# PRBonn/lidar_transfer

Measured on AMD Instinct MI355X. Metric: Mrays/sec, one new ~1M-triangle mesh per scan -> 64x2048 range/label image, higher is better.
Workload: dtype f32; 1 GPU; C2: 64x2048 rays vs 999788-triangle synthetic scene (fov 3.0/-25.0); 1 step = 64 scans, each a new mesh; 48 scenes cycled; parallelism=scan-parallel x1, scans_in_flight=24, scans_per_call=8

## Files before the change

### lidar_transfer_amd/csrc/lt_scatter.hip

```cpp
#include "lt_internal.h"
#include <math.h>
#include <stdlib.h>
#include <string.h>
#include "lt_normalize.h"

#define LT_PI_F 3.14159265358979f
#define LT_BIN_SLACK 4e-3f
#define LT_EMPTY_KEY 0xFFFFFFFFFFFFFFFFull

struct rs_params {
  int nb_az, nb_el;
  float az_scale;
  float az_off;
  float el_lo, el_scale;
  float dev_az, dev_el;
  float dev_fit[2];
  float el_c0, el_c1, az_c0, az_c1;
};

__device__ __forceinline__ float rs_az_off(float phi0, float az_scale) {
  if (!(phi0 == phi0)) return 0.f;
  const float x0 = (phi0 + LT_PI_F) * az_scale;
  return x0 - floorf(x0 + 0.5f);
}

__global__ __launch_bounds__(256) void k_rs_dirs(const float* __restrict__ rays, int n, unsigned flags,
                                                 float4* __restrict__ dirs, float2* __restrict__ ang,
                                                 float* __restrict__ partial) {
  __shared__ float red[4][2];
  float lo = INFINITY, hi = -INFINITY;
  for (int i = blockIdx.x * 256 + threadIdx.x; i < n; i += gridDim.x * 256) {
    const float rx = rays[3 * (size_t)i], ry = rays[3 * (size_t)i + 1], rz = rays[3 * (size_t)i + 2];
    const float D = (rx * rx + ry * ry) + rz * rz;
    const float r0 = lt_rsqrt_seed(D, flags);
    const float r = (1.5f * r0) + (((D * -0.5f) * r0) * (r0 * r0));
    const float dx = rx * r, dy = ry * r, dz = rz * r;
    dirs[i] = make_float4(dx, dy, dz, 0.f);
    const float phi = atan2f(dy, dx), th = atan2f(dz, sqrtf(dx * dx + dy * dy));
    ang[i] = make_float2(phi, th);
    if (th == th) { lo = fminf(lo, th); hi = fmaxf(hi, th); }
  }
#pragma unroll
  for (int o = 32; o > 0; o >>= 1) {
    lo = fminf(lo, __shfl_xor(lo, o, 64));
    hi = fmaxf(hi, __shfl_xor(hi, o, 64));
  }
  if ((threadIdx.x & 63) == 0) { red[threadIdx.x >> 6][0] = lo; red[threadIdx.x >> 6][1] = hi; }
  __syncthreads();
  if (threadIdx.x == 0) {
    partial[2 * blockIdx.x] = fminf(fminf(red[0][0], red[1][0]), fminf(red[2][0], red[3][0]));
    partial[2 * blockIdx.x + 1] = fmaxf(fmaxf(red[0][1], red[1][1]), fmaxf(red[2][1], red[3][1]));
  }
}

__global__ __launch_bounds__(256) void k_rs_fit(const float2* __restrict__ ang, int n, int nb_az0,
                                                rs_params* __restrict__ prm) {
  const float phi0 = n > 0 ? ang[0].x : 0.f;
  float dev[2] = {0.f, 0.f};
  for (int k = 0; k < 2; ++k) {
    const int K = nb_az0 - k;
    if (K < 1) continue;
    const float sc = (float)K / (2.0f * LT_PI_F), off = rs_az_off(phi0, sc);
    for (int i = blockIdx.x * 256 + threadIdx.x; i < n; i += gridDim.x * 256) {
      const float phi = ang[i].x;
      if (phi == phi) {
        const float x = (phi + LT_PI_F) * sc - off;
        dev[k] = fmaxf(dev[k], fabsf(x - floorf(x + 0.5f)));
      }
    }
  }
#pragma unroll
  for (int o = 32; o > 0; o >>= 1) {
    dev[0] = fmaxf(dev[0], __shfl_xor(dev[0], o, 64));
    dev[1] = fmaxf(dev[1], __shfl_xor(dev[1], o, 64));
  }
  if ((threadIdx.x & 63) == 0) {
    atomicMax((int*)&prm->dev_fit[0], __float_as_int(dev[0]));
    atomicMax((int*)&prm->dev_fit[1], __float_as_int(dev[1]));
  }
}

__global__ __launch_bounds__(256) void k_rs_keys(const float2* __restrict__ ang, int n, int nb_az, int nb_el, int refit,
                                                 const float* __restrict__ partial, rs_params* __restrict__ prm,
                                                 uint32_t* __restrict__ keys, uint32_t* __restrict__ vals) {
  __shared__ float red[4][2];
  float lo = partial[2 * threadIdx.x], hi = partial[2 * threadIdx.x + 1];
#pragma unroll
  for (int o = 32; o > 0; o >>= 1) {
    lo = fminf(lo, __shfl_xor(lo, o, 64));
    hi = fmaxf(hi, __shfl_xor(hi, o, 64));
  }
  if ((threadIdx.x & 63) == 0) { red[threadIdx.x >> 6][0] = lo; red[threadIdx.x >> 6][1] = hi; }
  __syncthreads();
  lo = fminf(fminf(red[0][0], red[1][0]), fminf(red[2][0], red[3][0]));
  hi = fmaxf(fmaxf(red[0][1], red[1][1]), fmaxf(red[2][1], red[3][1]));
  if (!(lo <= hi)) { lo = 0.f; hi = 0.f; }
  const int nb_max = nb_az;
  if (refit && nb_az >= 5 && prm->dev_fit[1] + 0.01f < prm->dev_fit[0]) nb_az -= 1;
  rs_params p;
  p.nb_az = nb_az; p.nb_el = nb_el;
  p.az_scale = (float)nb_az / (2.0f * LT_PI_F);
  p.az_off = rs_az_off(n > 0 ? ang[0].x : 0.f, p.az_scale);
  p.el_lo = lo;
  p.el_scale = (nb_el > 1 && hi > lo) ? (float)(nb_el - 1) / (hi - lo) : 0.f;
  if (blockIdx.x == 0 && threadIdx.x == 0) {
    prm->nb_az = p.nb_az; prm->nb_el = p.nb_el;
    prm->az_scale = p.az_scale; prm->az_off = p.az_off; prm->el_lo = p.el_lo; prm->el_scale = p.el_scale;
  }
  const int i = blockIdx.x * 256 + threadIdx.x;
  float dev_a = 0.f, dev_e = 0.f;
  if (i < n) {
    const float2 a = ang[i];
    uint32_t key = (uint32_t)nb_max * (uint32_t)nb_el;
    if (a.x == a.x && a.y == a.y) {
      const float x = (a.x + LT_PI_F) * p.az_scale - p.az_off, y = (a.y - p.el_lo) * p.el_scale;
      const float cx = floorf(x + 0.5f);
      const float cy = fminf(fmaxf(floorf(y + 0.5f), 0.f), (float)(nb_el - 1));
      dev_a = fabsf(x - cx);
      dev_e = fabsf(y - cy);
      int ia = (int)cx;
      if (ia < 0) ia += nb_az;
      else if (ia >= nb_az) ia -= nb_az;
      ia = min(max(ia, 0), nb_az - 1);
      key = (uint32_t)cy * (uint32_t)nb_az + (uint32_t)ia;
    }
    keys[i] = key;
    vals[i] = (uint32_t)i;
  }
#pragma unroll
  for (int o = 32; o > 0; o >>= 1) {
    dev_a = fmaxf(dev_a, __shfl_xor(dev_a, o, 64));
    dev_e = fmaxf(dev_e, __shfl_xor(dev_e, o, 64));
  }
  if ((threadIdx.x & 63) == 0) {
    atomicMax((int*)&prm->dev_az, __float_as_int(dev_a));
    atomicMax((int*)&prm->dev_el, __float_as_int(dev_e));
  }
}

__global__ __launch_bounds__(256) void k_rs_starts(const uint32_t* __restrict__ keys, int n, int nbins,
                                                   int* __restrict__ bin_start) {
  const int p = blockIdx.x * 256 + threadIdx.x;
  if (p > n) return;
  const int lo = p == 0 ? 0 : (int)min(keys[p - 1], (uint32_t)nbins) + 1;
  const int hi = p == n ? nbins : (int)min(keys[p], (uint32_t)nbins);
  for (int b = lo; b <= hi; ++b) bin_start[b] = p;
}

struct tri_rec {
  float v0x, v0y, v0z, e1x, e1y, e1z, e2x, e2y, e2z;
};

__device__ __forceinline__ float sc_mt(const tri_rec& T, float ox, float oy, float oz, float dx, float dy, float dz) {
  const float eps = 0.000001f;
  const float hx = dy * T.e2z - dz * T.e2y, hy = dz * T.e2x - dx * T.e2z, hz = dx * T.e2y - dy * T.e2x;
  const float a = (T.e1x * hx + T.e1y * hy) + T.e1z * hz;
  if (a < eps && a > -eps) return NAN;
  const float inv_a = lt_rcp_ieee(a);
  const float sx = ox - T.v0x, sy = oy - T.v0y, sz = oz - T.v0z;
  const float u = ((sx * hx + sy * hy) + sz * hz) * inv_a;
  if (u < 0 || u > 1) return NAN;
  const float qx = sy * T.e1z - sz * T.e1y, qy = sz * T.e1x - sx * T.e1z, qz = sx * T.e1y - sy * T.e1x;
  const float v = ((dx * qx + dy * qy) + dz * qz) * inv_a;
  if (v < 0 || u + v > 1) return NAN;
  const float t = ((T.e2x * qx + T.e2y * qy) + T.e2z * qz) * inv_a;
  if (t < eps) return NAN;
  return t;
}

__device__ __forceinline__ float f_rcp(float x) { return __builtin_amdgcn_rcpf(x); }
__device__ __forceinline__ float f_sqrt(float x) { return __builtin_amdgcn_sqrtf(x); }
__device__ __forceinline__ float f_atan2(float y, float x) {
#pragma clang fp contract(fast)
  const float ax = fabsf(x), ay = fabsf(y);
  const float mx = fmaxf(ax, ay), mn = fminf(ax, ay);
  const float a = mx > 0.f ? mn * f_rcp(mx) : 0.f;
  const float q = a * a;
  float r = a * (0.99997726f + q * (-0.33262347f + q * (0.19354346f + q * (-0.11643287f + q * (0.05265332f + q * -0.01172120f)))));
  r = ay > ax ? 1.57079632679f - r : r;
  r = x < 0.f ? 3.14159265359f - r : r;
  return y < 0.f ? -r : r;
}

__device__ __forceinline__ void f_atan_pair(float za, float ra, float zb, float rb, float& tha, float& thb) {
#pragma clang fp contract(fast)
  const float ta = za * f_rcp(ra), tb = zb * f_rcp(rb);
  const bool easy = fabsf(ta) <= 1.0f && fabsf(tb) <= 1.0f;
  if (__ballot(!easy) == 0ull) {
    const float qa = ta * ta, qb = tb * tb;
    tha = ta * (0.99997726f + qa * (-0.33262347f + qa * (0.19354346f + qa * (-0.11643287f + qa * (0.05265332f + qa * -0.01172120f)))));
    thb = tb * (0.99997726f + qb * (-0.33262347f + qb * (0.19354346f + qb * (-0.11643287f + qb * (0.05265332f + qb * -0.01172120f)))));
  } else {
    tha = f_atan2(za, ra);
    thb = f_atan2(zb, rb);
  }
}

__device__ __forceinline__ float seg_dist2d_sq(float ax, float ay, float bx, float by) {
#pragma clang fp contract(fast)
  const float ex = bx - ax, ey = by - ay;
  const float l2 = ex * ex + ey * ey;
  float t = l2 > 0.f ? -(ax * ex + ay * ey) * f_rcp(l2) : 0.f;
  t = fminf(fmaxf(t, 0.f), 1.f);
  const float cx = ax + t * ex, cy = ay + t * ey;
  return cx * cx + cy * cy;
}

template <class T>
__device__ __forceinline__ unsigned byte_off(unsigned elem) {
  if (sizeof(T) == 12) {
    unsigned r;
    asm("v_lshl_add_u32 %0, %1, 3, %2" : "=v"(r) : "v"(elem), "v"(elem << 2));
    return r;
  }
  return elem * (unsigned)sizeof(T);
}
template <bool WIDE, class T>
__device__ __forceinline__ const T* at(const T* base, unsigned elem) {
  return WIDE ? base + (size_t)elem : (const T*)((const char*)base + byte_off<T>(elem));
}
template <bool WIDE, class T>
__device__ __forceinline__ T* at(T* base, unsigned elem) {
  return WIDE ? base + (size_t)elem : (T*)((char*)base + byte_off<T>(elem));
}
struct f3 { float x, y, z; };
struct i3 { int x, y, z; };

struct bin_rect { int a0, na, e0, e1; };

__device__ __forceinline__ bin_rect tri_bins(const rs_params& P, float x0, float y0, float z0, float x1, float y1,
                                             float z1, float x2, float y2, float z2, float e1x, float e1y, float e2x,
                                             float e2y) {
#pragma clang fp contract(fast)
  bin_rect R;
  R.na = 0;
  const float q0 = x0 * x0 + y0 * y0, q1 = x1 * x1 + y1 * y1, q2 = x2 * x2 + y2 * y2;
  if (!(q0 + q1 + q2 < 1e36f && fabsf(z0) + fabsf(z1) + fabsf(z2) < 1e18f)) {
    const float sum = ((x0 + y0) + (z0 + x1)) + ((y1 + z1) + (x2 + y2)) + z2;
    const float asum = ((fabsf(x0) + fabsf(y0)) + (fabsf(z0) + fabsf(x1))) + ((fabsf(y1) + fabsf(z1)) + (fabsf(x2) + fabsf(y2))) + fabsf(z2);
    if (sum != sum || asum == INFINITY) return R;
    R.e0 = 0; R.e1 = P.nb_el - 1; R.a0 = 0; R.na = P.nb_az;
    return R;
  }
  const float rho_max2 = fmaxf(q0, fmaxf(q1, q2));
  const float rho_max = f_sqrt(rho_max2);
  const float zmin = fminf(z0, fminf(z1, z2)), zmax = fmaxf(z0, fmaxf(z1, z2));
  const float c0 = x0 * y1 - x1 * y0, c1 = x1 * y2 - x2 * y1, c2 = x2 * y0 - x0 * y2;
  const float tol = 1e-6f * rho_max2 + 1e-12f;
  const float cmin = fminf(c0, fminf(c1, c2)), cmax = fmaxf(c0, fmaxf(c1, c2));
  const bool outside = cmin < -tol && cmax > tol;
  bool edge_on = cmin >= -tol && cmax <= tol;
  const float e12x = e2x - e1x, e12y = e2y - e1y;
  const float lmax2 = fmaxf(e1x * e1x + e1y * e1y, fmaxf(e12x * e12x + e12y * e12y, e2x * e2x + e2y * e2y));
  const float qmin = fminf(q0, fminf(q1, q2));
  float rho_edges2;
  if (__ballot(!(lmax2 <= 0.01f * qmin)) == 0ull) {
    rho_edges2 = qmin - 0.25f * lmax2;
  } else {
    rho_edges2 =
        fminf(seg_dist2d_sq(x0, y0, x1, y1), fminf(seg_dist2d_sq(x1, y1, x2, y2), seg_dist2d_sq(x2, y2, x0, y0)));
  }
  const float rho_edges = f_sqrt(rho_edges2);
  const float rho_tiny = 1e-4f * rho_max + 1e-6f;
  if (!outside && rho_edges2 > 4.0f * lmax2) edge_on = true;
  const bool pierced = !(outside || (edge_on && rho_edges > rho_tiny));
  const float rho_min = pierced ? 0.f : rho_edges;
  const float z_near = __builtin_amdgcn_fmed3f(zmin, 0.f, zmax);
  const float dlo2 = fmaxf((pierced ? 0.f : rho_edges2) + z_near * z_near, 0.0025f);
  const float pad = 3e-4f + 2e-4f * __builtin_amdgcn_rsqf(dlo2);
  const float pad_az = 3e-4f + 2e-4f * __builtin_amdgcn_rsqf(fmaxf(rho_edges2, 0.0025f));
  float th_hi, th_lo;
  f_atan_pair(zmax, zmax > 0.f ? rho_min : rho_max, zmin, zmin < 0.f ? rho_min : rho_max, th_hi, th_lo);
  th_hi += pad;
  th_lo -= pad;
  const float fe0 = ceilf(th_lo * P.el_scale + P.el_c0), fe1 = floorf(th_hi * P.el_scale + P.el_c1);
  if (!(fe1 >= 0.f) || !(fe0 <= (float)(P.nb_el - 1)) || !(fe0 <= fe1)) return R;
  R.e0 = (int)fmaxf(fe0, 0.f);
  R.e1 = (int)fminf(fe1, (float)(P.nb_el - 1));
  if (pierced || rho_min <= rho_tiny || P.nb_az < 4) {
    R.a0 = 0;
    R.na = P.nb_az;
    return R;
  }
  float a_lo, a_hi;
  if (!edge_on) {
    const bool l0 = c0 >= 0.f && c2 <= 0.f, l1 = c1 >= 0.f && c0 <= 0.f;
    const bool h0 = c0 <= 0.f && c2 >= 0.f, h1 = c1 <= 0.f && c0 >= 0.f;
    a_lo = f_atan2(l0 ? y0 : (l1 ? y1 : y2), l0 ? x0 : (l1 ? x1 : x2));
    a_hi = f_atan2(h0 ? y0 : (h1 ? y1 : y2), h0 ? x0 : (h1 ? x1 : x2));
    if (a_hi < a_lo) a_hi += 2.0f * LT_PI_F;
  } else {
    const float p0 = f_atan2(y0, x0), p1 = f_atan2(y1, x1), p2 = f_atan2(y2, x2);
    const float lo = fminf(p0, fminf(p1, p2)), hi = fmaxf(p0, fmaxf(p1, p2));
    const float mid = (p0 + p1 + p2) - lo - hi;
    const float g0 = mid - lo, g1 = hi - mid, g2 = 2.0f * LT_PI_F - (hi - lo);
    if (g2 >= g0 && g2 >= g1) { a_lo = lo; a_hi = hi; }
    else if (g0 >= g1) { a_lo = mid; a_hi = lo + 2.0f * LT_PI_F; }
    else { a_lo = hi; a_hi = mid + 2.0f * LT_PI_F; }
  }
  a_lo -= pad_az;
  a_hi += pad_az;
  const float fa0 = ceilf(a_lo * P.az_scale + P.az_c0);
  const float fa1 = floorf(a_hi * P.az_scale + P.az_c1);
  const int na = (int)(fa1 - fa0) + 1;
  if (!(na >= 1)) return R;
  if (na >= P.nb_az) { R.a0 = 0; R.na = P.nb_az; return R; }
  int a0 = (int)fa0;
  if (a0 < 0) a0 += P.nb_az;
  else if (a0 >= P.nb_az) a0 -= P.nb_az;
  R.a0 = a0;
  R.na = na;
  return R;
}

#define LT_GRID_EMPTY (-1)
#define LT_GRID_MULTI (-2)
template <bool WIDE>
__device__ __forceinline__ void sc_hit(float t, int ray, int face, unsigned long long* __restrict__ cell) {
  if (t < 999999999.f) atomicMin(at<WIDE>(cell, (unsigned)ray), ((unsigned long long)__float_as_uint(t) << 32) | (unsigned)face);
}
template <bool WIDE>
__device__ __forceinline__ void sc_test_cell(const tri_rec& T, int face, const float4 g,
                                             const float4* __restrict__ sdirs, float ox, float oy, float oz,
                                             unsigned long long* __restrict__ cell, unsigned& n_tests) {
  const int w = __float_as_int(g.w);
  if (w != LT_GRID_MULTI) {
    n_tests += w >= 0 ? 1u : 0u;
    sc_hit<WIDE>(sc_mt(T, ox, oy, oz, g.x, g.y, g.z), w, face, cell);
  } else {
    for (int k = __float_as_int(g.x), e = __float_as_int(g.y); k < e; ++k) {
      const float4 d = *at<WIDE>(sdirs, (unsigned)k);
      ++n_tests;
      sc_hit<WIDE>(sc_mt(T, ox, oy, oz, d.x, d.y, d.z), __float_as_int(d.w), face, cell);
    }
  }
}

__global__ __launch_bounds__(256) void k_rs_sortdirs(const float4* __restrict__ dirs,
                                                     const uint32_t* __restrict__ bin_rays, int n,
                                                     float4* __restrict__ sdirs) {
  const int k = blockIdx.x * 256 + threadIdx.x;
  if (k >= n) return;
  const int ray = (int)bin_rays[k];
  float4 d = dirs[ray];
  d.w = __int_as_float(ray);
  sdirs[k] = d;
}

__global__ __launch_bounds__(256) void k_rs_grid(const int* __restrict__ bin_start,
                                                 const float4* __restrict__ sdirs, int nbins,
                                                 float4* __restrict__ grid) {
  const int b = blockIdx.x * 256 + threadIdx.x;
  if (b >= nbins) return;
  const int s = bin_start[b], e = bin_start[b + 1];
  float4 g = make_float4(0.f, 0.f, 0.f, __int_as_float(LT_GRID_EMPTY));
  if (e - s == 1) g = sdirs[s];
  else if (e - s > 1) g = make_float4(__int_as_float(s), __int_as_float(e), 0.f, __int_as_float(LT_GRID_MULTI));
  grid[b] = g;
}

#define LT_SC_BIG 512
#define LT_SC_CAP_SINGLE 1536
#define LT_SC_CAP_BATCH 8192
#ifndef LT_SC_SLICE
#define LT_SC_SLICE 512
#endif

#ifndef LT_SC_T
#define LT_SC_T 448
#endif
#define LT_SC_T2 (LT_SC_T - 256)
static_assert(LT_SC_T >= 256 && LT_SC_T <= 512 && LT_SC_T2 % 64 == 0, "LT_SC_T: 256, 320, 384, 448 or 512");

struct sc_shared {
  float4 q0[LT_SC_T], q1[LT_SC_T];
  float2 q2[LT_SC_T];
  unsigned pre[513];
  unsigned wsum[4];
  int kept;
};

struct sc_one { int cnt; unsigned a0; };

template <bool PUSH>
__device__ __forceinline__ sc_one sc_record_into(float4* s_q0, float4* s_q1, float2* s_q2, int slot, int f, const f3 A,
                                                 const f3 Bv, const f3 C, float ox, float oy, float oz, const rs_params& P,
                                                 int* __restrict__ large, int* __restrict__ large_count) {
  sc_one r;
  r.cnt = 0; r.a0 = 0;
  const float v0x = A.x, v0y = A.y, v0z = A.z, v1x = Bv.x, v1y = Bv.y, v1z = Bv.z;
  const float v2x = C.x, v2y = C.y, v2z = C.z;
  const float e1x = v1x - v0x, e1y = v1y - v0y, e2x = v2x - v0x, e2y = v2y - v0y;
  const bin_rect R = tri_bins(P, v0x - ox, v0y - oy, v0z - oz, v1x - ox, v1y - oy, v1z - oz, v2x - ox, v2y - oy,
                              v2z - oz, e1x, e1y, e2x, e2y);
  if (R.na > 0) {
    const int c32 = R.na * (R.e1 - R.e0 + 1);
    if (c32 > LT_SC_BIG) {
      if (PUSH) large[atomicAdd(large_count, 1)] = f;
    } else {
      r.cnt = c32;
      r.a0 = (unsigned)R.a0;
      s_q0[slot] = make_float4(v0x, v0y, v0z, e1x);
      s_q1[slot] = make_float4(e1y, v1z - v0z, e2x, e2y);
      s_q2[slot] = make_float2(v2z - v0z, __int_as_float((R.na - 1) | (R.e0 << 9)));
    }
  }
  return r;
}
template <bool PUSH>
__device__ __forceinline__ sc_one sc_record(sc_shared& S, int slot, int f, const f3 A, const f3 Bv, const f3 C, float ox,
                                            float oy, float oz, const rs_params& P, int* __restrict__ large,
                                            int* __restrict__ large_count) {
  return sc_record_into<PUSH>(S.q0, S.q1, S.q2, slot, f, A, Bv, C, ox, oy, oz, P, large, large_count);
}

template <bool PUSH, bool WIDE>
__device__ __forceinline__ void sc_setup(sc_shared& S, const float* __restrict__ verts, const int* __restrict__ faces,
                                         int n_verts, int n_faces, int first, float ox, float oy, float oz,
                                         const rs_params& P, int* __restrict__ large, int* __restrict__ large_count,
                                         unsigned* __restrict__ flags, sc_one& rA, sc_one& rB) {
  const int tid = threadIdx.x;
  rA.cnt = 0; rA.a0 = 0; rB.cnt = 0; rB.a0 = 0;
  const int fA = first + tid, fB = first + 256 + tid;
  const bool hasA = fA < n_faces, hasB = LT_SC_T2 > 0 && tid < LT_SC_T2 && fB < n_faces;
  if (n_verts <= 0) {
    if (PUSH && (hasA || hasB)) atomicOr(flags, LT_FLAG_BAD_INDEX);
    return;
  }
  const i3 iA = *at<WIDE>((const i3*)faces, (unsigned)(hasA ? fA : 0));
  i3 iB = iA;
  if (LT_SC_T2 > 0) iB = *at<WIDE>((const i3*)faces, (unsigned)(hasB ? fB : 0));
  const unsigned nv = (unsigned)n_verts;
  const bool okA = hasA && (unsigned)iA.x < nv && (unsigned)iA.y < nv && (unsigned)iA.z < nv;
  const bool okB = hasB && (unsigned)iB.x < nv && (unsigned)iB.y < nv && (unsigned)iB.z < nv;
  const f3 A0 = *at<WIDE>((const f3*)verts, okA ? (unsigned)iA.x : 0u);
  const f3 A1 = *at<WIDE>((const f3*)verts, okA ? (unsigned)iA.y : 0u);
  const f3 A2 = *at<WIDE>((const f3*)verts, okA ? (unsigned)iA.z : 0u);
  f3 B0 = A0, B1 = A1, B2 = A2;
  if (LT_SC_T2 > 0) {
    B0 = *at<WIDE>((const f3*)verts, okB ? (unsigned)iB.x : 0u);
    B1 = *at<WIDE>((const f3*)verts, okB ? (unsigned)iB.y : 0u);
    B2 = *at<WIDE>((const f3*)verts, okB ? (unsigned)iB.z : 0u);
  }
  if (PUSH && ((hasA && !okA) || (hasB && !okB))) atomicOr(flags, LT_FLAG_BAD_INDEX);
  if (okA) rA = sc_record<PUSH>(S, tid, fA, A0, A1, A2, ox, oy, oz, P, large, large_count);
  if (LT_SC_T2 > 0 && okB) rB = sc_record<PUSH>(S, 256 + tid, fB, B0, B1, B2, ox, oy, oz, P, large, large_count);
}

__device__ __forceinline__ void sc_prefix(sc_shared& S, const sc_one rA, const sc_one rB, int& preA, int& preB, int& total) {
  const int tid = threadIdx.x, lane = tid & 63, wave = tid >> 6;
  unsigned inc = (unsigned)rA.cnt | ((unsigned)rB.cnt << 16);
  asm volatile(
      "s_nop 1\n\tv_add_u32_dpp %0, %0, %0 row_shr:1 row_mask:0xf bank_mask:0xf bound_ctrl:0\n\t"
      "s_nop 1\n\tv_add_u32_dpp %0, %0, %0 row_shr:2 row_mask:0xf bank_mask:0xf bound_ctrl:0\n\t"
      "s_nop 1\n\tv_add_u32_dpp %0, %0, %0 row_shr:4 row_mask:0xf bank_mask:0xf bound_ctrl:0\n\t"
      "s_nop 1\n\tv_add_u32_dpp %0, %0, %0 row_shr:8 row_mask:0xf bank_mask:0xf bound_ctrl:0\n\t"
      "s_nop 1\n\tv_add_u32_dpp %0, %0, %0 row_bcast:15 row_mask:0xa bank_mask:0xf\n\t"
      "s_nop 1\n\tv_add_u32_dpp %0, %0, %0 row_bcast:31 row_mask:0xc bank_mask:0xf\n\t"
      "s_nop 1"
      : "+v"(inc));
  if (lane == 63) S.wsum[wave] = inc;
  __syncthreads();
  int woffA = 0, woffB = 0, totA = 0, totB = 0;
#pragma unroll
  for (int w = 0; w < 4; ++w) {
    const unsigned ws = S.wsum[w];
    const int a = (int)(ws & 0xFFFFu), b = (int)(ws >> 16);
    if (w < wave) { woffA += a; woffB += b; }
    totA += a; totB += b;
  }
  total = totA + totB;
  preA = woffA + (int)(inc & 0xFFFFu) - rA.cnt;
  preB = totA + woffB + (int)(inc >> 16) - rB.cnt;
  S.pre[tid] = ((unsigned)preA << 13) | rA.a0;
  if (LT_SC_T2 > 0 && tid < LT_SC_T2) S.pre[256 + tid] = ((unsigned)preB << 13) | rB.a0;
  else S.pre[256 + tid] = (256 + tid == LT_SC_T) ? ((unsigned)total << 13) : 0xFFFFFFFFu;
  if (tid == 255) S.pre[512] = LT_SC_T == 512 ? ((unsigned)total << 13) : 0xFFFFFFFFu;
}

template <bool COUNT, bool WIDE, int NT, int NE>
__device__ __forceinline__ void sc_round_robin(const unsigned* s_pre, const float4* s_q0, const float4* s_q1,
                                               const float2* s_q2, const rs_params& P, const float4* __restrict__ grid,
                                               const float4* __restrict__ sdirs, unsigned long long* __restrict__ cell,
                                               int first_face, int c_begin, int c_end, int tix, float ox, float oy, float oz,
                                               unsigned& n_tests, unsigned& n_cand) {
  auto ldu = [](const unsigned* arr, unsigned j4) { return *(const unsigned*)((const char*)arr + j4); };
  auto ldq = [](const float4* arr, unsigned j4) { return *(const float4*)((const char*)arr + 4u * j4); };
  auto ld2 = [](const float2* arr, unsigned j4) { return *(const float2*)((const char*)arr + 2u * j4); };
  const unsigned pre0 = s_pre[0];
  auto locate = [&](int c, unsigned& j4, float2& q2) -> int {
    const unsigned ck = ((unsigned)c << 13) | 0x1FFFu;
    j4 = 0;
    unsigned base = pre0;
#pragma unroll
    for (unsigned step4 = 2u * NE; step4 >= 4; step4 >>= 1) {
      const unsigned v = ldu(s_pre, j4 + step4);
      const bool take = v <= ck;
      j4 = take ? j4 + step4 : j4;
      base = take ? v : base;
    }
    const int local = c - (int)(base >> 13);
    q2 = ld2(s_q2, j4);
    const int pk = __float_as_int(q2.y);
    const int na = (pk & 511) + 1;
    const int row = (int)(((float)local + 0.5f) * f_rcp((float)na));
    int az = (int)(base & 0x1FFFu) + (local - __mul24(row, na));
    if (az >= P.nb_az) az -= P.nb_az;
    return __mul24((pk >> 9) + row, P.nb_az) + az;
  };
  int c = c_begin + tix;
  if (c < c_end) {
    unsigned j4;
    float2 q2;
    float4 g = *at<false>(grid, (unsigned)locate(c, j4, q2));
    for (;;) {
      const int cn = c + NT;
      unsigned jn4 = 0;
      float2 q2n = make_float2(0.f, 0.f);
      float4 gn = make_float4(0.f, 0.f, 0.f, 0.f);
      if (__ballot(cn < c_end) != 0ull) gn = *at<false>(grid, (unsigned)locate(min(cn, c_end - 1), jn4, q2n));
      const float4 q0 = ldq(s_q0, j4), q1 = ldq(s_q1, j4);
      tri_rec T;
      T.v0x = q0.x; T.v0y = q0.y; T.v0z = q0.z;
      T.e1x = q0.w; T.e1y = q1.x; T.e1z = q1.y;
      T.e2x = q1.z; T.e2y = q1.w; T.e2z = q2.x;
      if (COUNT) ++n_cand;
      sc_test_cell<WIDE>(T, first_face + (int)(j4 >> 2), g, sdirs, ox, oy, oz, cell, n_tests);
      if (cn >= c_end) break;
      c = cn; j4 = jn4; g = gn; q2 = q2n;
    }
  }
}

template <bool COUNT>
__device__ __forceinline__ void sc_count(unsigned n_tests, unsigned n_cand, unsigned long long* __restrict__ counters) {
  if (COUNT) {
    unsigned long long vt = n_tests, vc = n_cand;
#pragma unroll
    for (int o = 32; o > 0; o >>= 1) { vt += __shfl_xor(vt, o, 64); vc += __shfl_xor(vc, o, 64); }
    if ((threadIdx.x & 63) == 0) { atomicAdd(&counters[1], vt); atomicAdd(&counters[0], vc); }
  }
}

#ifndef LT_SC_MAX_BATCH
#define LT_SC_MAX_BATCH 8
#endif
struct sc_job {
  const float* verts; const int* faces; const int* colors; const float* rem;
  rs_params P; const float4* grid; const float4* sdirs; const float4* dirs;
  unsigned long long* cell; int* large; int* large_count; int2* slices;
  unsigned* flags; unsigned long long* counters;
  float* endpoints; int* endcolors; float* range; float* endrem; int* tri;
  float ox, oy, oz;
  int n_verts, n_faces, n_rays, cap_slices;
  unsigned out_flags;
};
struct sc_batch {
  int n;
  int tris_blocks, resolve_blocks;
  int cap;
  int rest_blocks;
  int tris_block0[LT_SC_MAX_BATCH];
  int resolve_block0[LT_SC_MAX_BATCH];
  sc_job job[LT_SC_MAX_BATCH];
};
__device__ __forceinline__ int sc_find_job(const int (&block0)[LT_SC_MAX_BATCH], int block) {
  int j = 0;
#pragma unroll
  for (int k = 1; k < LT_SC_MAX_BATCH; ++k) j += block >= block0[k] ? 1 : 0;
  return j;
}


template <bool COUNT, bool WIDE>
__global__ __launch_bounds__(256) void k_sc_tris(const sc_batch B) {
  __shared__ sc_shared S;
  const int j = sc_find_job(B.tris_block0, (int)blockIdx.x);
  const sc_job& J = B.job[j];
  const int lb = (int)blockIdx.x - B.tris_block0[j];
  const int tid = threadIdx.x;
  const int first = lb * LT_SC_T;
  const rs_params P = J.P;
  const float ox = J.ox, oy = J.oy, oz = J.oz;
  sc_one rA, rB;
  sc_setup<true, WIDE>(S, J.verts, J.faces, J.n_verts, J.n_faces, first, ox, oy, oz, P, J.large, J.large_count, J.flags, rA,
                       rB);
  int total, preA, preB;
  sc_prefix(S, rA, rB, preA, preB, total);
  if (total < B.cap) {
    if (tid == 255) S.kept = total;
  } else {
    const bool crossA = preA < B.cap && preA + rA.cnt >= B.cap;
    const bool crossB = LT_SC_T2 > 0 && tid < LT_SC_T2 && preB < B.cap && preB + rB.cnt >= B.cap;
    if (crossA || crossB) {
      int kept = crossA ? preA + rA.cnt : preB + rB.cnt;
      const int n_sl = (total - kept + LT_SC_SLICE - 1) / LT_SC_SLICE;
      if (n_sl > 0) {
        const int base = atomicAdd(&J.large_count[1], n_sl);
        if (base + n_sl <= J.cap_slices) {
          for (int k = 0; k < n_sl; ++k) J.slices[base + k] = make_int2(lb, kept + k * LT_SC_SLICE);
        } else {
          atomicSub(&J.large_count[1], n_sl);
          kept = total;
        }
      }
      S.kept = kept;
    }
  }
  __syncthreads();
  const int kept = S.kept;
  unsigned n_tests = 0, n_cand = 0;
  sc_round_robin<COUNT, WIDE, 256, (LT_SC_T > 256 ? 512 : 256)>(S.pre, S.q0, S.q1, S.q2, P, J.grid, J.sdirs, J.cell, first, 0,
                                                                kept, tid, ox, oy, oz, n_tests, n_cand);
  sc_count<COUNT>(n_tests, n_cand, J.counters);
}

#define LT_SC_REST_BLOCKS 512
#define LT_SC_REST_BLOCKS_BATCH 128
#define LT_SC_PARTS 8
template <bool COUNT, bool WIDE>
__global__ __launch_bounds__(256) void k_sc_rest(const sc_batch B) {
  __shared__ sc_shared S;
  const int rest_blocks = B.rest_blocks;
  const sc_job& J = B.job[blockIdx.x / rest_blocks];
  const int rb = blockIdx.x % rest_blocks;
  if (J.n_faces <= 0) return;
  const float* __restrict__ verts = J.verts;
  const int* __restrict__ faces = J.faces;
  const float4* __restrict__ grid = J.grid;
  const float4* __restrict__ sdirs = J.sdirs;
  unsigned long long* __restrict__ cell = J.cell;
  const float ox = J.ox, oy = J.oy, oz = J.oz;
  const rs_params P = J.P;
  const int n_large = J.large_count[0], n_slices = min(J.large_count[1], J.cap_slices);
  if (COUNT && rb == 0 && threadIdx.x == 0) J.counters[3] = (unsigned long long)n_large | ((unsigned long long)n_slices << 32);
  unsigned n_tests = 0, n_cand = 0;
  for (int q = rb; q < n_slices; q += rest_blocks) {
    const int2 sl = J.slices[q];
    const int first = sl.x * LT_SC_T;
    sc_one rA, rB;
    sc_setup<false, WIDE>(S, verts, faces, J.n_verts, J.n_faces, first, ox, oy, oz, P, nullptr, nullptr, nullptr, rA, rB);
    int total, preA, preB;
    sc_prefix(S, rA, rB, preA, preB, total);
    __syncthreads();
    sc_round_robin<COUNT, WIDE, 256, (LT_SC_T > 256 ? 512 : 256)>(S.pre, S.q0, S.q1, S.q2, P, grid, sdirs, cell, first, sl.y,
                                                                  min(sl.y + LT_SC_SLICE, total), (int)threadIdx.x, ox, oy,
                                                                  oz, n_tests, n_cand);
    __syncthreads();
  }
  const int lane = threadIdx.x & 63;
  const int wave0 = rb * 4 + (threadIdx.x >> 6), nwaves = rest_blocks * 4;
  for (int v = wave0; v < n_large * LT_SC_PARTS; v += nwaves) {
    const int q = v / LT_SC_PARTS, part = v - q * LT_SC_PARTS;
    const int f = J.large[q];
    const float* pa = verts + 3 * (size_t)faces[3 * (size_t)f];
    const float* pb = verts + 3 * (size_t)faces[3 * (size_t)f + 1];
    const float* pc = verts + 3 * (size_t)faces[3 * (size_t)f + 2];
    tri_rec T;
    T.v0x = pa[0]; T.v0y = pa[1]; T.v0z = pa[2];
    const float v1x = pb[0], v1y = pb[1], v1z = pb[2], v2x = pc[0], v2y = pc[1], v2z = pc[2];
    T.e1x = v1x - T.v0x; T.e1y = v1y - T.v0y; T.e1z = v1z - T.v0z;
    T.e2x = v2x - T.v0x; T.e2y = v2y - T.v0y; T.e2z = v2z - T.v0z;
    const bin_rect R = tri_bins(P, T.v0x - ox, T.v0y - oy, T.v0z - oz, v1x - ox, v1y - oy, v1z - oz, v2x - ox,
                                v2y - oy, v2z - oz, T.e1x, T.e1y, T.e2x, T.e2y);
    const int total = R.na > 0 ? R.na * (R.e1 - R.e0 + 1) : 0;
    const int parts = min(max((total + 1023) / 1024, 1), LT_SC_PARTS);
    if (part >= parts) continue;
    for (int w = part * 64 + lane; w < total; w += 64 * parts) {
      const int row = w / R.na;
      const int e = R.e0 + row;
      int az = R.a0 + (w - row * R.na);
      if (az >= P.nb_az) az -= P.nb_az;
      if (COUNT) ++n_cand;
      sc_test_cell<WIDE>(T, f, grid[e * P.nb_az + az], sdirs, ox, oy, oz, cell, n_tests);
    }
  }
  sc_count<COUNT>(n_tests, n_cand, J.counters);
}

template <bool COUNT>
__global__ __launch_bounds__(256) void k_sc_resolve(const sc_batch B) {
  const int j = sc_find_job(B.resolve_block0, (int)blockIdx.x);
  const sc_job& J = B.job[j];
  const int ray = ((int)blockIdx.x - B.resolve_block0[j]) * 256 + threadIdx.x;
  unsigned long long* __restrict__ cell = J.cell;
  const int* __restrict__ faces = J.faces;
  float* __restrict__ endpoints = J.endpoints;
  int* __restrict__ endcolors = J.endcolors;
  float* __restrict__ range = J.range;
  float* __restrict__ endrem = J.endrem;
  int* __restrict__ tri_out = J.tri;
  const unsigned flags = J.out_flags;
  if (ray == 0) { J.large_count[0] = 0; J.large_count[1] = 0; }
  bool hit = false;
  if (ray < J.n_rays) {
    const unsigned long long key = cell[ray];
    const float4 d = J.dirs[ray];
    cell[ray] = LT_EMPTY_KEY;
    hit = key != LT_EMPTY_KEY;
    if (hit) {
      const float t = __uint_as_float((unsigned)(key >> 32));
      const int face = (int)(unsigned)(key & 0xFFFFFFFFull);
      const int i0 = faces[3 * (size_t)face], i1 = faces[3 * (size_t)face + 1], i2 = faces[3 * (size_t)face + 2];
      const int* __restrict__ colors = J.colors;
      const float* __restrict__ rem = J.rem;
      const bool label = (flags & LT_TRACE_LABEL_IMAGE) != 0;
      int c0 = 0, c1 = 0, c2 = 0;
      float r0 = 0.f, r1 = 0.f, r2 = 0.f;
      if (endcolors) {
        c2 = colors[3 * (size_t)i0 + 2];
        if (!label) { c0 = colors[3 * (size_t)i0]; c1 = colors[3 * (size_t)i0 + 1]; }
      }
      if (endrem) { r0 = rem[i0]; r1 = rem[i1]; r2 = rem[i2]; }
      if (endpoints) {
        endpoints[3 * (size_t)ray] = J.ox + d.x * t;
        endpoints[3 * (size_t)ray + 1] = J.oy + d.y * t;
        endpoints[3 * (size_t)ray + 2] = J.oz + d.z * t;
      }
      if (endcolors) {
        if (label) {
          endcolors[ray] = (int)(float)c2;
        } else {
          endcolors[3 * (size_t)ray] = (int)(float)c0;
          endcolors[3 * (size_t)ray + 1] = (int)(float)c1;
          endcolors[3 * (size_t)ray + 2] = (int)(float)c2;
        }
      }
      if (endrem) endrem[ray] = ((r0 + r1) + r2) / 3.0f;
      if (range) range[ray] = t;
      if (tri_out) tri_out[ray] = face;
    } else if (flags & LT_TRACE_WRITE_MISSES) {
      if (endpoints) { endpoints[3 * (size_t)ray] = 0.f; endpoints[3 * (size_t)ray + 1] = 0.f; endpoints[3 * (size_t)ray + 2] = 0.f; }
      if (endcolors) {
        if (flags & LT_TRACE_LABEL_IMAGE) endcolors[ray] = 0;
        else { endcolors[3 * (size_t)ray] = 0; endcolors[3 * (size_t)ray + 1] = 0; endcolors[3 * (size_t)ray + 2] = 0; }
      }
      if (endrem) endrem[ray] = 0.f;
      if (range) range[ray] = 0.f;
      if (tri_out) tri_out[ray] = -1;
    }
  }
  if (COUNT) {
    unsigned long long vh = hit ? 1u : 0u;
#pragma unroll
    for (int o = 32; o > 0; o >>= 1) vh += __shfl_xor(vh, o, 64);
    if ((threadIdx.x & 63) == 0) atomicAdd(&J.counters[2], vh);
  }
}

void lt_sort_pairs(uint32_t* keys[2], uint32_t* vals[2], uint32_t* hist, int n, int key_bits, hipStream_t stream,
                   int* out_buffer);

static void rs_derive(rs_params& p) {
  const float de = p.dev_el + LT_BIN_SLACK, da = p.dev_az + LT_BIN_SLACK;
  p.el_c0 = -p.el_lo * p.el_scale - de;
  p.el_c1 = -p.el_lo * p.el_scale + de;
  p.az_c0 = LT_PI_F * p.az_scale - p.az_off - da;
  p.az_c1 = LT_PI_F * p.az_scale - p.az_off + da;
}

struct lt_rayset {
  int device;
  int n_rays, height, nb_az, nb_el;
  unsigned norm_flags;
  float4* dirs;
  float2* ang;
  float* partial;
  rs_params* prm;
  rs_params prm_host;
  uint32_t* keys[2];
  uint32_t* vals[2];
  uint32_t* hist;
  int* bin_start;
  uint32_t* bin_rays;
  float4* sdirs;
  float4* grid;
};

static void rs_free(lt_rayset* r) {
  void* ps[] = {r->grid, r->sdirs, r->dirs, r->ang, r->partial, r->prm, r->keys[0], r->keys[1], r->vals[0], r->vals[1], r->hist,
                r->bin_start};
  for (void* p : ps)
    if (p) (void)hipFree(p);
}

extern "C" int lt_rayset_destroy(lt_rayset* r) {
  if (!r) return LT_OK;
  (void)hipSetDevice(r->device);
  (void)hipDeviceSynchronize();
  rs_free(r);
  free(r);
  return LT_OK;
}

static int rs_create(const char* who, lt_rayset** out, const float* rays, int n_rays, int height, int grid_az, int grid_el,
                     unsigned flags, void* stream_) {
  if (!out || n_rays < 0 || height <= 0 || grid_az < 0 || grid_el < 0 || (n_rays > 0 && !rays)) {
    lt_set_error("%s: invalid argument (n_rays=%d height=%d nb_az=%d nb_el=%d)", who, n_rays, height, grid_az, grid_el);
    return LT_ERR_INVALID_ARG;
  }
  *out = nullptr;
  hipStream_t stream = (hipStream_t)stream_;
  int device = 0;
  LT_HIP(hipGetDevice(&device));
  lt_rayset* r = (lt_rayset*)calloc(1, sizeof(lt_rayset));
  if (!r) return LT_ERR_NO_MEMORY;
  r->device = device;
  const int W = n_rays / height;
  const int n = W * height;
  r->n_rays = n;
  r->height = height;
  r->norm_flags = flags & (LT_TRACE_NORM_EXACT | LT_TRACE_NORM_AMD);
  const int want_az = grid_az > 0 ? grid_az : W, want_el = grid_el > 0 ? grid_el : height;
  r->nb_az = want_az < 1 ? 1 : (want_az > 8192 ? 8192 : want_az);
  r->nb_el = want_el > 4096 ? 4096 : want_el;
  const size_t nbins = (size_t)r->nb_az * r->nb_el + 1;
  const size_t nn = n > 0 ? n : 1;
  const int nb = (int)((nn + LT_SORT_TILE - 1) / LT_SORT_TILE);
  int rc = LT_OK;
#define RS_ALLOC(ptr, bytes)                                                  \
  if (rc == LT_OK && hipMalloc((void**)&(ptr), (bytes)) != hipSuccess) {      \
    lt_set_error("%s: hipMalloc of %zu bytes failed", who, (size_t)(bytes)); \
    rc = LT_ERR_NO_MEMORY;                                                    \
  }
  RS_ALLOC(r->dirs, nn * sizeof(float4));
  RS_ALLOC(r->ang, nn * sizeof(float2));
  RS_ALLOC(r->sdirs, nn * sizeof(float4));
  RS_ALLOC(r->partial, 2 * 256 * sizeof(float));
  RS_ALLOC(r->prm, sizeof(rs_params));
  for (int k = 0; k < 2; ++k) {
    RS_ALLOC(r->keys[k], nn * sizeof(uint32_t));
    RS_ALLOC(r->vals[k], nn * sizeof(uint32_t));
  }
  RS_ALLOC(r->hist, ((size_t)1024 * nb + 1024) * sizeof(uint32_t));
  RS_ALLOC(r->bin_start, (nbins + 1) * sizeof(int));
  RS_ALLOC(r->grid, nbins * sizeof(float4));
#undef RS_ALLOC
  if (rc != LT_OK) {
    rs_free(r);
    free(r);
    return rc;
  }
  if (hipMemsetAsync(r->prm, 0, sizeof(rs_params), stream) != hipSuccess) {
    lt_set_error("%s: hipMemsetAsync failed", who);
    rs_free(r);
    free(r);
    return LT_ERR_HIP;
  }
  hipLaunchKernelGGL(k_rs_dirs, dim3(256), dim3(256), 0, stream, rays, n, r->norm_flags, r->dirs, r->ang, r->partial);
  const int refit = grid_az > 0 ? 0 : 1;
  if (refit) hipLaunchKernelGGL(k_rs_fit, dim3(64), dim3(256), 0, stream, r->ang, n, r->nb_az, r->prm);
  hipLaunchKernelGGL(k_rs_keys, dim3((n + 255) / 256 > 0 ? (n + 255) / 256 : 1), dim3(256), 0, stream, r->ang, n,
                     r->nb_az, r->nb_el, refit, r->partial, r->prm, r->keys[0], r->vals[0]);
  int buf = 0;
  if (n > 0) lt_sort_pairs(r->keys, r->vals, r->hist, n, 30, stream, &buf);
  r->bin_rays = r->vals[buf];
  hipLaunchKernelGGL(k_rs_starts, dim3((n + 1 + 255) / 256), dim3(256), 0, stream, r->keys[buf], n, (int)nbins,
                     r->bin_start);
  if (n > 0)
    hipLaunchKernelGGL(k_rs_sortdirs, dim3((n + 255) / 256), dim3(256), 0, stream, r->dirs, r->bin_rays, n, r->sdirs);
  hipLaunchKernelGGL(k_rs_grid, dim3((unsigned)((nbins + 255) / 256)), dim3(256), 0, stream, r->bin_start, r->sdirs,
                     (int)nbins, r->grid);
  const hipError_t le = hipGetLastError();
  if (le != hipSuccess) {
    lt_set_error("%s: kernel launch failed: %s", who, hipGetErrorString(le));
    (void)hipStreamSynchronize(stream);
    rs_free(r);
    free(r);
    return LT_ERR_HIP;
  }
  if (hipStreamSynchronize(stream) != hipSuccess ||
      hipMemcpy(&r->prm_host, r->prm, sizeof(rs_params), hipMemcpyDeviceToHost) != hipSuccess) {
    lt_set_error("%s: ray set preparation failed: %s", who, hipGetErrorString(hipGetLastError()));
    rs_free(r);
    free(r);
    return LT_ERR_HIP;
  }
  rs_derive(r->prm_host);
  *out = r;
  return LT_OK;
}

extern "C" int lt_rayset_create_dev(lt_rayset** out, const float* rays, int n_rays, int height, unsigned flags,
                                    void* stream) {
  return rs_create("lt_rayset_create_dev", out, rays, n_rays, height, 0, 0, flags, stream);
}

extern "C" int lt_rayset_create_grid_dev(lt_rayset** out, const float* rays, int n_rays, int height, int nb_az, int nb_el,
                                         unsigned flags, void* stream) {
  return rs_create("lt_rayset_create_grid_dev", out, rays, n_rays, height, nb_az, nb_el, flags, stream);
}

static int sc_reserve(lt_scene* s, int n_faces, int n_rays, hipStream_t stream) {
  if (!s->sc_large_count) {
    LT_HIP(hipMalloc((void**)&s->sc_large_count, 4 * sizeof(int)));
    LT_HIP(hipMemsetAsync(s->sc_large_count, 0, 4 * sizeof(int), stream));
  }
  if (n_rays > s->sc_cap_cells) {
    if (s->sc_cell) {
      LT_HIP(hipDeviceSynchronize());
      (void)hipFree(s->sc_cell);
      s->sc_cell = nullptr;
      s->sc_cap_cells = 0;
    }
    LT_HIP(hipMalloc((void**)&s->sc_cell, (size_t)n_rays * sizeof(unsigned long long)));
    s->sc_cap_cells = n_rays;
    LT_HIP(hipMemsetAsync(s->sc_cell, 0xFF, (size_t)n_rays * sizeof(unsigned long long), stream));
  }
  if (n_faces > s->sc_cap_queue) {
    if (s->sc_large || s->sc_slices) {
      LT_HIP(hipDeviceSynchronize());
      (void)hipFree(s->sc_large);
      (void)hipFree(s->sc_slices);
      s->sc_large = nullptr;
      s->sc_slices = nullptr;
      s->sc_cap_queue = 0;
    }
    const size_t cap = (size_t)n_faces + n_faces / 4 + 1024;
    LT_HIP(hipMalloc((void**)&s->sc_large, cap * sizeof(int)));
    LT_HIP(hipMalloc((void**)&s->sc_slices, cap * sizeof(int2)));
    s->sc_cap_queue = (int)cap;
  }
  return LT_OK;
}

struct sc_item {
  lt_scene* s;
  lt_rayset* r;
  const float* origin;
  float* endpoints; int* endcolors; float* range; float* endrem; int* tri;
};

static int sc_launch_batch(const sc_item* it, int n_items, unsigned flags, hipStream_t stream, bool count,
                           lt_scene* probe) {
  sc_batch B;
  memset(&B, 0, sizeof(B));
  for (int k = 0; k < LT_SC_MAX_BATCH; ++k) B.tris_block0[k] = B.resolve_block0[k] = 0x7fffffff;
  static const bool force_wide = getenv("LIDARHIP_FORCE_WIDE") != nullptr;
  bool wide = force_wide;
  int tb = 0, rb = 0;
  for (int i = 0; i < n_items; ++i) {
    lt_scene* s = it[i].s;
    lt_rayset* r = it[i].r;
    const int n = s->n_faces, R = r->n_rays;
    if (R <= 0) continue;
    LT_CHECK(sc_reserve(s, n, R, stream));
    sc_job& J = B.job[B.n++];
    J.verts = s->verts; J.faces = s->faces; J.colors = s->colors; J.rem = s->rem;
    J.P = r->prm_host; J.grid = r->grid; J.sdirs = r->sdirs; J.dirs = r->dirs;
    J.cell = s->sc_cell; J.large = s->sc_large; J.large_count = s->sc_large_count; J.slices = s->sc_slices;
    J.flags = s->flags; J.counters = s->counters;
    J.endpoints = it[i].endpoints; J.endcolors = it[i].endcolors; J.range = it[i].range; J.endrem = it[i].endrem;
    J.tri = it[i].tri;
    J.ox = it[i].origin[0]; J.oy = it[i].origin[1]; J.oz = it[i].origin[2];
    J.n_verts = s->n_verts; J.n_faces = n; J.n_rays = R; J.cap_slices = s->sc_cap_queue;
    J.out_flags = flags;
    B.tris_block0[B.n - 1] = tb;
    B.resolve_block0[B.n - 1] = rb;
    tb += (n + LT_SC_T - 1) / LT_SC_T;
    rb += (R + 255) / 256;
    wide = wide || (size_t)n * 12 >= (1ull << 32) || (size_t)s->n_verts * 12 >= (1ull << 32) ||
           (size_t)R * 16 >= (1ull << 32);
  }
  if (B.n == 0) return LT_OK;
  B.tris_blocks = tb;
  B.resolve_blocks = rb;
  static const int env_cap = []() {
    const char* e = getenv("LIDARHIP_SC_CAP");
    return e ? atoi(e) : 0;
  }();
  B.cap = env_cap > 0 ? env_cap : (n_items > 1 ? LT_SC_CAP_BATCH : LT_SC_CAP_SINGLE);
  static const int env_rest = []() {
    const char* e = getenv("LIDARHIP_SC_REST_BLOCKS");
    return e ? atoi(e) : 0;
  }();
  B.rest_blocks = env_rest > 0 ? env_rest : (n_items > 1 ? LT_SC_REST_BLOCKS_BATCH : LT_SC_REST_BLOCKS);
  const dim3 b(256);
#define SC_LAUNCH(KERNEL, GRID) \
  do { \
    if (count && wide) hipLaunchKernelGGL((KERNEL<true, true>), GRID, b, 0, stream, B); \
    else if (count) hipLaunchKernelGGL((KERNEL<true, false>), GRID, b, 0, stream, B); \
    else if (wide) hipLaunchKernelGGL((KERNEL<false, true>), GRID, b, 0, stream, B); \
    else hipLaunchKernelGGL((KERNEL<false, false>), GRID, b, 0, stream, B); \
  } while (0)
  if (tb > 0) {
    if (probe && probe->probe[0]) LT_HIP(hipEventRecord(probe->probe[0], stream));
    SC_LAUNCH(k_sc_tris, dim3(tb));
    if (probe) {
      if (probe->probe[1]) LT_HIP(hipEventRecord(probe->probe[1], stream));
      probe->probe[0] = probe->probe[1] = nullptr;
    }
    SC_LAUNCH(k_sc_rest, dim3(B.n * B.rest_blocks));
  }
#undef SC_LAUNCH
  if (count) hipLaunchKernelGGL(k_sc_resolve<true>, dim3(rb), b, 0, stream, B);
  else hipLaunchKernelGGL(k_sc_resolve<false>, dim3(rb), b, 0, stream, B);
  LT_HIP(hipGetLastError());
  return LT_OK;
}

extern "C" int lt_scene_render_dev(lt_scene* s, lt_rayset* r, const float* origin, float* endpoints, int* endcolors,
                                   float* range, float* endrem, int* tri, unsigned flags, void* stream_,
                                   lt_stats* stats) {
  if (!s || !r || !origin) {
    lt_set_error("lt_scene_render_dev: NULL scene / rayset / origin");
    return LT_ERR_INVALID_ARG;
  }
  if (s->device != r->device) {
    lt_set_error("lt_scene_render_dev: scene on device %d, rayset on device %d", s->device, r->device);
    return LT_ERR_INVALID_ARG;
  }
  hipStream_t stream = (hipStream_t)stream_;
  LT_HIP(hipSetDevice(s->device));
  s->last_stream = stream;
  const int n = s->n_faces, R = r->n_rays;
  const bool timed = stats != nullptr, count = (flags & LT_TRACE_COUNT) != 0;
  s->stats.n_rays = R;
  s->stats.n_faces = n;
  if (R > 0) {
    if (count) LT_HIP(hipMemsetAsync(s->counters, 0, 4 * sizeof(unsigned long long), stream));
    if (timed) LT_HIP(hipEventRecord(s->ev[7], stream));
    const sc_item it = {s, r, origin, endpoints, endcolors, range, endrem, tri};
    LT_CHECK(sc_launch_batch(&it, 1, flags, stream, count, count ? nullptr : s));
    if (timed) LT_HIP(hipEventRecord(s->ev[8], stream));
  }
  if (timed || count) {
    LT_HIP(hipStreamSynchronize(stream));
    if (timed && R > 0) LT_HIP(hipEventElapsedTime(&s->stats.ms_trace, s->ev[7], s->ev[8]));
    if (count && R > 0) {
      unsigned long long c[4];
      LT_HIP(hipMemcpy(c, s->counters, sizeof(c), hipMemcpyDeviceToHost));
      s->stats.nodes_visited = c[0];
      s->stats.tris_tested = c[1];
      s->stats.n_hits = (int)c[2];
      s->stats.stack_overflows = 0;
      s->stats.entries_culled = 0;
    }
    if (stats) *stats = s->stats;
  }
  return LT_OK;
}

extern "C" int lt_scene_render_batch_dev(int n_scans, lt_scene* const* scenes, lt_rayset* const* raysets,
                                         const float* origins, float* const* endpoints, int* const* endcolors,
                                         float* const* range, float* const* endrem, int* const* tri, unsigned flags,
                                         void* stream_) {
  if (n_scans < 0 || n_scans > LT_SC_MAX_BATCH || (n_scans > 0 && (!scenes || !raysets || !origins))) {
    lt_set_error("lt_scene_render_batch_dev: invalid argument (n_scans=%d, at most %d per call)", n_scans,
                 LT_SC_MAX_BATCH);
    return LT_ERR_INVALID_ARG;
  }
  if (flags & LT_TRACE_COUNT) {
    lt_set_error("lt_scene_render_batch_dev: LT_TRACE_COUNT is a single-scan diagnostic (lt_scene_render_dev)");
    return LT_ERR_INVALID_ARG;
  }
  if (n_scans == 0) return LT_OK;
  hipStream_t stream = (hipStream_t)stream_;
  sc_item it[LT_SC_MAX_BATCH];
  lt_scene* probe = nullptr;
  for (int i = 0; i < n_scans; ++i) {
    if (!scenes[i] || !raysets[i] || scenes[i]->device != raysets[i]->device ||
        scenes[i]->device != scenes[0]->device) {
      lt_set_error("lt_scene_render_batch_dev: scan %d: NULL scene / rayset, or not all on one device", i);
      return LT_ERR_INVALID_ARG;
    }
    for (int k = 0; k < i; ++k)
      if (scenes[k] == scenes[i]) {
        lt_set_error("lt_scene_render_batch_dev: scans %d and %d are the same scene (a scene renders one scan at a time)", k, i);
        return LT_ERR_INVALID_ARG;
      }
    it[i] = {scenes[i], raysets[i], origins + 3 * i, endpoints ? endpoints[i] : nullptr,
             endcolors ? endcolors[i] : nullptr, range ? range[i] : nullptr, endrem ? endrem[i] : nullptr,
             tri ? tri[i] : nullptr};
    scenes[i]->last_stream = stream;
    scenes[i]->stats.n_rays = raysets[i]->n_rays;
    scenes[i]->stats.n_faces = scenes[i]->n_faces;
    if (!probe && scenes[i]->probe[0]) probe = scenes[i];
  }
  LT_HIP(hipSetDevice(scenes[0]->device));
  return sc_launch_batch(it, n_scans, flags, stream, false, probe ? probe : scenes[0]);
}

extern "C" int lt_debug_scatter_queues(lt_scene* s, int* out2) {
  if (!s || !out2) return LT_ERR_INVALID_ARG;
  LT_HIP(hipSetDevice(s->device));
  LT_HIP(hipDeviceSynchronize());
  unsigned long long c = 0;
  LT_HIP(hipMemcpy(&c, s->counters + 3, sizeof(c), hipMemcpyDeviceToHost));
  out2[0] = (int)(c & 0xFFFFFFFFull);
  out2[1] = (int)(c >> 32);
  return LT_OK;
}
extern "C" int lt_debug_scatter_large(lt_scene* s, int* out, int n) {
  if (!s || !out || n < 0 || n > s->sc_cap_queue) return LT_ERR_INVALID_ARG;
  LT_HIP(hipSetDevice(s->device));
  LT_HIP(hipDeviceSynchronize());
  LT_HIP(hipMemcpy(out, s->sc_large, (size_t)n * sizeof(int), hipMemcpyDeviceToHost));
  return LT_OK;
}
extern "C" int lt_debug_rayset_params(lt_rayset* r, int* nb, float* p) {
  if (!r || !nb || !p) return LT_ERR_INVALID_ARG;
  const rs_params& P = r->prm_host;
  nb[0] = P.nb_az; nb[1] = P.nb_el;
  p[0] = P.az_scale; p[1] = P.az_off; p[2] = P.el_lo; p[3] = P.el_scale; p[4] = P.dev_az; p[5] = P.dev_el;
  return LT_OK;
}
```

Baseline: 11730 Mrays/s.

## Batch several candidate cells per thread in scatter round-robin for memory-level parallelism

```diff
diff --git a/lidar_transfer_amd/csrc/lt_scatter.hip b/lidar_transfer_amd/csrc/lt_scatter.hip
--- a/lidar_transfer_amd/csrc/lt_scatter.hip
+++ b/lidar_transfer_amd/csrc/lt_scatter.hip
@@ -1,5 +1,6 @@
 #include "lt_internal.h"
 #include <math.h>
+#include <type_traits>
 #include <stdlib.h>
 #include <string.h>
 #include "lt_normalize.h"
@@ -478,7 +479,15 @@
   if (tid == 255) S.pre[512] = LT_SC_T == 512 ? ((unsigned)total << 13) : 0xFFFFFFFFu;
 }
 
-template <bool COUNT, bool WIDE, int NT, int NE>
+#ifndef LT_SC_PB
+#define LT_SC_PB 3
+#endif
+static_assert(LT_SC_PB >= 1 && LT_SC_PB <= 4, "LT_SC_PB: 1 .. 4");
+#ifndef LT_SC_PB_REST
+#define LT_SC_PB_REST 1
+#endif
+static_assert(LT_SC_PB_REST >= 1 && LT_SC_PB_REST <= 4, "LT_SC_PB_REST: 1 .. 4");
+template <bool COUNT, bool WIDE, int NT, int NE, int PB>
 __device__ __forceinline__ void sc_round_robin(const unsigned* s_pre, const float4* s_q0, const float4* s_q1,
                                                const float2* s_q2, const rs_params& P, const float4* __restrict__ grid,
                                                const float4* __restrict__ sdirs, unsigned long long* __restrict__ cell,
@@ -488,19 +497,8 @@
   auto ldq = [](const float4* arr, unsigned j4) { return *(const float4*)((const char*)arr + 4u * j4); };
   auto ld2 = [](const float2* arr, unsigned j4) { return *(const float2*)((const char*)arr + 2u * j4); };
   const unsigned pre0 = s_pre[0];
-  auto locate = [&](int c, unsigned& j4, float2& q2) -> int {
-    const unsigned ck = ((unsigned)c << 13) | 0x1FFFu;
-    j4 = 0;
-    unsigned base = pre0;
-#pragma unroll
-    for (unsigned step4 = 2u * NE; step4 >= 4; step4 >>= 1) {
-      const unsigned v = ldu(s_pre, j4 + step4);
-      const bool take = v <= ck;
-      j4 = take ? j4 + step4 : j4;
-      base = take ? v : base;
-    }
+  auto bin_of = [&](int c, unsigned base, const float2 q2) -> int {
     const int local = c - (int)(base >> 13);
-    q2 = ld2(s_q2, j4);
     const int pk = __float_as_int(q2.y);
     const int na = (pk & 511) + 1;
     const int row = (int)(((float)local + 0.5f) * f_rcp((float)na));
@@ -508,27 +506,66 @@
     if (az >= P.nb_az) az -= P.nb_az;
     return __mul24((pk >> 9) + row, P.nb_az) + az;
   };
-  int c = c_begin + tix;
-  if (c < c_end) {
-    unsigned j4;
-    float2 q2;
-    float4 g = *at<false>(grid, (unsigned)locate(c, j4, q2));
-    for (;;) {
-      const int cn = c + NT;
-      unsigned jn4 = 0;
-      float2 q2n = make_float2(0.f, 0.f);
-      float4 gn = make_float4(0.f, 0.f, 0.f, 0.f);
-      if (__ballot(cn < c_end) != 0ull) gn = *at<false>(grid, (unsigned)locate(min(cn, c_end - 1), jn4, q2n));
-      const float4 q0 = ldq(s_q0, j4), q1 = ldq(s_q1, j4);
+  auto block = [&](auto n_tag, const int cb) {
+    constexpr int N = decltype(n_tag)::value;
+    int cc[N];
+    unsigned ck[N], j4[N], base[N];
+#pragma unroll
+    for (int u = 0; u < N; ++u) {
+      cc[u] = min(cb + u * NT, c_end - 1);
+      ck[u] = ((unsigned)cc[u] << 13) | 0x1FFFu;
+      j4[u] = 0;
+      base[u] = pre0;
+    }
+#pragma unroll
+    for (unsigned step4 = 2u * NE; step4 >= 4; step4 >>= 1) {
+#pragma unroll
+      for (int u = 0; u < N; ++u) {
+        const unsigned v = ldu(s_pre, j4[u] + step4);
+        const bool take = v <= ck[u];
+        j4[u] = take ? j4[u] + step4 : j4[u];
+        base[u] = take ? v : base[u];
+      }
+    }
+    float2 q2[N];
+#pragma unroll
+    for (int u = 0; u < N; ++u) q2[u] = ld2(s_q2, j4[u]);
+    float4 g[N];
+#pragma unroll
+    for (int u = 0; u < N; ++u) g[u] = *at<false>(grid, (unsigned)bin_of(cc[u], base[u], q2[u]));
+    float th[N];
+#pragma unroll
+    for (int u = 0; u < N; ++u) {
+      const bool act = cb + u * NT < c_end;
+      const float4 q0 = ldq(s_q0, j4[u]), q1 = ldq(s_q1, j4[u]);
       tri_rec T;
       T.v0x = q0.x; T.v0y = q0.y; T.v0z = q0.z;
       T.e1x = q0.w; T.e1y = q1.x; T.e1z = q1.y;
-      T.e2x = q1.z; T.e2y = q1.w; T.e2z = q2.x;
-      if (COUNT) ++n_cand;
-      sc_test_cell<WIDE>(T, first_face + (int)(j4 >> 2), g, sdirs, ox, oy, oz, cell, n_tests);
-      if (cn >= c_end) break;
-      c = cn; j4 = jn4; g = gn; q2 = q2n;
-    }
+      T.e2x = q1.z; T.e2y = q1.w; T.e2z = q2[u].x;
+      const int w = __float_as_int(g[u].w);
+      if (COUNT) n_cand += act ? 1u : 0u;
+      n_tests += act && w >= 0 ? 1u : 0u;
+      const float t = sc_mt(T, ox, oy, oz, g[u].x, g[u].y, g[u].z);
+      th[u] = act && w != LT_GRID_MULTI ? t : NAN;
+      if (act && w == LT_GRID_MULTI) sc_test_cell<WIDE>(T, first_face + (int)(j4[u] >> 2), g[u], sdirs, ox, oy, oz, cell, n_tests);
+    }
+#pragma unroll
+    for (int u = 0; u < N; ++u) sc_hit<WIDE>(th[u], __float_as_int(g[u].w), first_face + (int)(j4[u] >> 2), cell);
+  };
+  for (int cb = c_begin + tix; cb < c_end; cb += PB * NT) {
+    int live = 1;
+#pragma unroll
+    for (int u = 1; u < PB; ++u) live += __ballot(cb + u * NT < c_end) != 0ull ? 1 : 0;
+    if constexpr (PB >= 4) {
+      if (live == 4) { block(std::integral_constant<int, 4>{}, cb); continue; }
+    }
+    if constexpr (PB >= 3) {
+      if (live == 3) { block(std::integral_constant<int, 3>{}, cb); continue; }
+    }
+    if constexpr (PB >= 2) {
+      if (live == 2) { block(std::integral_constant<int, 2>{}, cb); continue; }
+    }
+    block(std::integral_constant<int, 1>{}, cb);
   }
 }
 
@@ -610,8 +647,8 @@
   __syncthreads();
   const int kept = S.kept;
   unsigned n_tests = 0, n_cand = 0;
-  sc_round_robin<COUNT, WIDE, 256, (LT_SC_T > 256 ? 512 : 256)>(S.pre, S.q0, S.q1, S.q2, P, J.grid, J.sdirs, J.cell, first, 0,
-                                                                kept, tid, ox, oy, oz, n_tests, n_cand);
+  sc_round_robin<COUNT, WIDE, 256, (LT_SC_T > 256 ? 512 : 256), LT_SC_PB>(S.pre, S.q0, S.q1, S.q2, P, J.grid, J.sdirs, J.cell,
+                                                                          first, 0, kept, tid, ox, oy, oz, n_tests, n_cand);
   sc_count<COUNT>(n_tests, n_cand, J.counters);
 }
 
@@ -643,9 +680,9 @@
     int total, preA, preB;
     sc_prefix(S, rA, rB, preA, preB, total);
     __syncthreads();
-    sc_round_robin<COUNT, WIDE, 256, (LT_SC_T > 256 ? 512 : 256)>(S.pre, S.q0, S.q1, S.q2, P, grid, sdirs, cell, first, sl.y,
-                                                                  min(sl.y + LT_SC_SLICE, total), (int)threadIdx.x, ox, oy,
-                                                                  oz, n_tests, n_cand);
+    sc_round_robin<COUNT, WIDE, 256, (LT_SC_T > 256 ? 512 : 256), LT_SC_PB_REST>(S.pre, S.q0, S.q1, S.q2, P, grid, sdirs, cell,
+                                                                               first, sl.y, min(sl.y + LT_SC_SLICE, total),
+                                                                               (int)threadIdx.x, ox, oy, oz, n_tests, n_cand);
     __syncthreads();
   }
   const int lane = threadIdx.x & 63;
```

Measured after the change: 11960 Mrays/s, median of 6. 1.02x the previous value.
